# argmaxinc/WhisperKit

Measured on NVIDIA H100. Metric: RTFx (audio-sec/s) whisper-large-v3 greedy, higher is better.
Workload: dtype bf16

## Files before the change

### include/wkb200.h

```cpp
#ifndef WKB200_H
#define WKB200_H

#include <stdint.h>

#ifdef __cplusplus
extern "C" {
#endif

typedef int32_t wk_status;
enum {
    WK_OK = 0,
    WK_ERR_INVALID_ARGUMENT = -1,
    WK_ERR_MODELS_UNAVAILABLE = -2,
    WK_ERR_AUDIO_PROCESSING_FAILED = -3,
    WK_ERR_PREPARE_DECODER_INPUTS = -4,
    WK_ERR_DECODING_LOGITS_FAILED = -5,
    WK_ERR_DECODING_FAILED = -6,
    WK_ERR_TRANSCRIPTION_FAILED = -7,
    WK_ERR_CUDA = -8
};

typedef struct wk_model wk_model;
typedef struct wk_session wk_session;
typedef struct wk_tensor wk_tensor;
// ... 250 lines not shown
int32_t wk_write_srt(const float* starts, const float* ends, const char* const* texts, int32_t n, char* out, int32_t cap);
int32_t wk_write_vtt(const float* starts, const float* ends, const char* const* texts, int32_t n, char* out, int32_t cap);

int64_t wk_kernel_launch_count(int32_t reset);
wk_status wk_last_timings(wk_model* m, float* ms6);
void* wk_model_stream(wk_model* m);

wk_status wk_test_gemm(wk_model* m, const void* a, const void* w, const float* bias, void* out, int32_t M, int32_t N, int32_t K,
                       int32_t in_dtype, int32_t out_dtype, int32_t gelu);
wk_status wk_test_gemm_residual(wk_model* m, const void* a, const void* w, const float* bias, float* out, int32_t M, int32_t N, int32_t K, int32_t in_dtype);
wk_status wk_test_gemm_splitk(wk_model* m, const void* w, const void* x, float* out, int32_t N, int32_t rows_x, int32_t K, int32_t in_dtype, int32_t splits);
wk_status wk_test_attention(wk_model* m, const void* qkv, void* out, int32_t B, int32_t T, int32_t n_heads, int32_t dtype);
wk_status wk_test_cross_attention(wk_model* m, const float* q, const void* kcross, const void* vcross, void* out, int32_t B, int32_t H,
                                  int32_t T, int32_t dtype, const int32_t* done);
wk_status wk_test_cross_attention_shared(wk_model* m, const float* q, const void* kcross, const void* vcross, void* out, int32_t B, int32_t H,
                                         int32_t T, int32_t dtype, const int32_t* done, int32_t kv_div);
wk_status wk_test_cross_attention_fp8(wk_model* m, const float* q, const uint8_t* kcodes, const uint8_t* vcodes, const float* kscale,
                                      const float* vscale, void* out, int32_t B, int32_t H, int32_t T, int32_t dtype, const int32_t* done,
                                      int32_t kv_div, float* align_out);
wk_status wk_test_self_attention(wk_model* m, const float* qkv, void* kcache, void* vcache, const int32_t* pos, void* out, int32_t B,
                                 int32_t H, int32_t dtype, const int32_t* done);
wk_status wk_test_gemm_partial(wk_model* m, const void* w, const void* x, float* partial_out, int32_t N, int32_t rows_x, int32_t partial_cols,
                               int32_t K, int32_t dtype, int32_t splits);
wk_status wk_test_decoder_reduce(wk_model* m, int32_t kind, const float* partial, int32_t splits, int32_t Bp, const float* bias, const float* gamma,
                                 const float* beta, float* x, void* out16, int32_t B, int32_t n, int32_t dtype);
wk_status wk_test_self_attention_splitk(wk_model* m, const float* partial, int32_t splits, int32_t Bp, const float* bq, const float* bv, void* kcache,
                                        void* vcache, const int32_t* pos, const int32_t* done, const int32_t* anc, void* out, int32_t B, int32_t H,
                                        int32_t dtype);
wk_status wk_test_cross_attention_splitk(wk_model* m, const float* partial, int32_t splits, int32_t Bp, const float* bq, const void* kcross,
                                         const void* vcross, const float* kscale, const float* vscale, void* out, int32_t B, int32_t H, int32_t T,
                                         int32_t dtype, const int32_t* done, int32_t kv_div);

wk_status wk_bench_kernel(wk_model* m, wk_session* s, int32_t which, int32_t batch, int32_t iters, float* ms_out, double* work_out);

wk_status wk_debug_read(wk_model* m, wk_session* s, int32_t which, int64_t offset_elems, float* dst, int64_t n);

#ifdef __cplusplus
}
#endif
#endif
```

### whisperkit_b200/_lib.py

```python
from __future__ import annotations

import ctypes as C
import os

_PKG = os.path.dirname(os.path.abspath(__file__))
LIB_PATH = os.path.join(_PKG, "libwkb200.so")

WK_DTYPE_F32, WK_DTYPE_F16, WK_DTYPE_BF16, WK_DTYPE_I32 = 0, 1, 2, 3
WK_DTYPE_FP8_E4M3 = 4

STATUS_NAMES = {
    0: "ok", -1: "invalidArgument", -2: "modelsUnavailable", -3: "audioProcessingFailed",
    -4: "prepareDecoderInputsFailed", -5: "decodingLogitsFailed", -6: "decodingFailed",
    -7: "transcriptionFailed", -8: "cudaError",
}


class WhisperError(RuntimeError):

    def __init__(self, status: int, message: str):
        super().__init__(f"{STATUS_NAMES.get(status, status)}: {message}")
        self.status = status
        self.case = STATUS_NAMES.get(status, str(status))

# ... 172 lines not shown
    ("wk_tokenizer_vocab_size", I32, [P]),
    ("wk_tokenizer_token_to_id", I32, [P, C.c_char_p]),
    ("wk_tokenizer_decode", I32, [P, PI32, I32, I32, C.POINTER(C.c_char), I32]),
    ("wk_tokenizer_encode", I32, [P, C.c_char_p, PI32, I32]),
    ("wk_tokenizer_set_merges", I32, [P, C.POINTER(C.c_char_p), C.POINTER(C.c_char_p), I32]),
    ("wk_tokenizer_special_tokens", I32, [P, C.POINTER(wk_special_tokens)]),
    ("wk_tokenizer_split_to_word_tokens", I32, [P, PI32, I32, C.POINTER(C.c_char), I32, PI32, I32]),
    ("wk_tokenizer_hooks_init", I32, [P, C.POINTER(wk_tokenizer_hooks)]),
    ("wk_format_time", I32, [F32, I32, C.c_char_p, C.POINTER(C.c_char), I32]),
    ("wk_write_srt", I32, [PF32, PF32, C.POINTER(C.c_char_p), I32, C.POINTER(C.c_char), I32]),
    ("wk_write_vtt", I32, [PF32, PF32, C.POINTER(C.c_char_p), I32, C.POINTER(C.c_char), I32]),
    ("wk_kernel_launch_count", I64, [I32]),
    ("wk_last_timings", I32, [P, PF32]),
    ("wk_model_stream", P, [P]),
    ("wk_test_gemm", I32, [P, P, P, P, P, I32, I32, I32, I32, I32, I32]),
    ("wk_test_cross_attention", I32, [P, P, P, P, P, I32, I32, I32, I32, P]),
    ("wk_test_cross_attention_shared", I32, [P, P, P, P, P, I32, I32, I32, I32, P, I32]),
    ("wk_test_cross_attention_fp8", I32, [P, P, P, P, P, P, P, I32, I32, I32, I32, P, I32, P]),
    ("wk_test_self_attention", I32, [P, P, P, P, P, P, I32, I32, I32, P]),
    ("wk_test_gemm_residual", I32, [P, P, P, P, P, I32, I32, I32, I32]),
    ("wk_test_gemm_splitk", I32, [P, P, P, P, I32, I32, I32, I32, I32]),
    ("wk_test_attention", I32, [P, P, P, I32, I32, I32, I32]),
    ("wk_test_gemm_partial", I32, [P, P, P, P, I32, I32, I32, I32, I32, I32]),
    ("wk_test_decoder_reduce", I32, [P, I32, P, I32, I32, P, P, P, P, P, I32, I32, I32]),
    ("wk_test_self_attention_splitk", I32, [P, P, I32, I32, P, P, P, P, P, P, P, P, I32, I32, I32]),
    ("wk_test_cross_attention_splitk", I32, [P, P, I32, I32, P, P, P, P, P, P, I32, I32, I32, I32, P, I32]),
    ("wk_debug_read", I32, [P, P, I32, I64, P, I64]),
    ("wk_bench_kernel", I32, [P, P, I32, I32, I32, PF32, C.POINTER(C.c_double)]),
]

_lib = None


def load() -> C.CDLL:
    global _lib
    if _lib is not None:
        return _lib
    if not os.path.exists(LIB_PATH):
        raise ImportError(
            f"{LIB_PATH} not built: run `python -m whisperkit_b200.build` (needs nvcc). "
            "whisperkit_b200 has no CPU or PyTorch fallback.")
    lib = C.CDLL(LIB_PATH)
    for name, restype, argtypes in SYMBOLS:
        fn = getattr(lib, name)
        fn.restype = restype
        fn.argtypes = argtypes
# ... 8 lines not shown
```

### whisperkit_b200/csrc/decoder_ops.cu

```cuda
#include <curand_kernel.h>
#include <math.h>

#include <stdlib.h>

#include "common.cuh"
#include <algorithm>
#include "kernels.h"

namespace wk {

static constexpr int kMaxCtx = 224;

__device__ __forceinline__ float block_sum(float v, float* scratch) {
    v = warp_sum(v);
    const int warp = threadIdx.x >> 5, lane = threadIdx.x & 31, nw = (blockDim.x + 31) >> 5;
    __syncthreads();
    if (lane == 0) scratch[warp] = v;
    __syncthreads();
    float r = (lane < nw) ? scratch[lane] : 0.f;
    r = warp_sum(r);
    return r;
}
__device__ __forceinline__ float block_max(float v, float* scratch) {
    v = warp_max(v);
// ... 586 lines not shown
    launch_k(decoder_cross_attention_kernel<T, FP8>, dim3(B * H), dim3(kCrossThreads), cross_smem_bytes<FP8>(Tlen), stream, 4, partial, splits, Bp, bq,
             (const uint8_t*)kcross, (const uint8_t*)vcross, kscale, vscale, (T*)out, B, H, Tlen, done, align_scratch, align_mask, kv_div);
    return WK_OK;
}


__global__ void decoder_align_mean_kernel(const float* __restrict__ scratch, int n_slots, const int32_t* __restrict__ steps,
                                          const int32_t* __restrict__ done, const int32_t* __restrict__ lang_state, __half* __restrict__ out,
                                          int B, int Tlen, int max_rows) {
    const int b = blockIdx.y, t = blockIdx.x * blockDim.x + threadIdx.x;
    const int row = steps[b];
    if (t >= Tlen || row >= max_rows || done[b] || (lang_state != nullptr && lang_state[b] == kLangLeadRan)) return;
    float a = 0.f;
    for (int s = 0; s < n_slots; ++s) a += scratch[((long long)s * B + b) * Tlen + t];
    out[((long long)b * max_rows + row) * Tlen + t] = __float2half(a / (float)n_slots);
}

wk_status decoder_align_mean(const float* scratch, int n_slots, const int32_t* steps, const int32_t* done, const int32_t* lang_state,
                             void* out_f16, int B, int T, int max_rows, cudaStream_t stream) {
    launch_k(decoder_align_mean_kernel, dim3((T + 255) / 256, B), dim3(256), 0, stream, 0, scratch, n_slots, steps, done, lang_state, (__half*)out_f16, B, T, max_rows);
    count_launch();
    cudaError_t e = cudaGetLastError();
    if (e != cudaSuccess) { set_error("decoder_align_mean launch: %s", cudaGetErrorString(e)); return WK_ERR_CUDA; }
    return WK_OK;
}

wk_status decoder_cross_attention(const float* partial, int splits, int Bp, const float* bq, const void* kcross,
                                  const void* vcross, void* out, int B, int H, int T, int dtype, cudaStream_t stream,
                                  const int32_t* done, float* align_scratch, uint32_t align_mask, int kv_div, const float* kscale,
                                  const float* vscale) {
    const bool fp8 = kscale != nullptr;
    if (kv_div < 1 || B % kv_div != 0) { set_error("decoder_cross_attention: %d rows do not split into groups of %d", B, kv_div); return WK_ERR_INVALID_ARGUMENT; }
    if (!fp8 && T % kCrossRows != 0) { set_error("decoder_cross_attention: n_audio_ctx %d not a multiple of %d", T, kCrossRows); return WK_ERR_INVALID_ARGUMENT; }
    if (kv_div > 1 && kv_div <= 8 && align_scratch == nullptr)
        return decoder_cross_attention_mq(partial, splits, Bp, bq, kcross, vcross, out, B, H, T, dtype, stream, done, kv_div, kscale, vscale);
    if (fp8 && (T % CrossCfg<true>::kRows != 0 || T % 4 != 0)) { set_error("decoder_cross_attention (fp8): n_audio_ctx %d not a multiple of 500", T); return WK_ERR_INVALID_ARGUMENT; }
    const bool f16 = dtype == WK_DTYPE_F16;
    wk_status st = fp8 ? (f16 ? launch_cross<__half, true>(partial, splits, Bp, bq, kcross, vcross, kscale, vscale, out, B, H, T, stream, done, align_scratch, align_mask, kv_div)
                              : launch_cross<__nv_bfloat16, true>(partial, splits, Bp, bq, kcross, vcross, kscale, vscale, out, B, H, T, stream, done, align_scratch, align_mask, kv_div))
                       : (f16 ? launch_cross<__half, false>(partial, splits, Bp, bq, kcross, vcross, kscale, vscale, out, B, H, T, stream, done, align_scratch, align_mask, kv_div)
                              : launch_cross<__nv_bfloat16, false>(partial, splits, Bp, bq, kcross, vcross, kscale, vscale, out, B, H, T, stream, done, align_scratch, align_mask, kv_div));
    if (st != WK_OK) return st;
    count_launch();
    cudaError_t e = cudaGetLastError();
    if (e != cudaSuccess) { set_error("decoder_cross_attention launch: %s", cudaGetErrorString(e)); return WK_ERR_CUDA; }
    return WK_OK;
// ... 457 lines not shown
```

### whisperkit_b200/csrc/engine.cu

```cuda
#include <math.h>
#include <stdarg.h>
#include <stdio.h>
#include <stdlib.h>
#include <string.h>
#include <dirent.h>

#include <algorithm>
#include <atomic>
#include <map>
#include <string>
#include <vector>

#include "common.cuh"
#include "engine.h"

namespace wk {

static thread_local char g_err[1024] = "";
void set_error(const char* fmt, ...) {
    va_list ap;
    va_start(ap, fmt);
    vsnprintf(g_err, sizeof(g_err), fmt, ap);
    va_end(ap);
}
// ... 1022 lines not shown

wk_status wk_test_gemm_partial(wk_model* m, const void* w, const void* x, float* partial_out, int32_t N, int32_t rows_x, int32_t partial_cols,
                               int32_t K, int32_t dtype, int32_t splits) {
    if (!m || !w || !x || !partial_out || N < 1 || rows_x < 16 || rows_x > 256 || rows_x % 16 != 0 || partial_cols < 1 || partial_cols > rows_x ||
        splits < 1) {
        set_error("wk_test_gemm_partial: bad arguments");
        return WK_ERR_INVALID_ARGUMENT;
    }
    WK_CUDA_CHECK(cudaSetDevice(m->device));
    std::lock_guard<std::mutex> lock(m->api_mu);
    GemmDesc g;
    memset(&g, 0, sizeof(g));
    g.a = w; g.a_rows = N; g.a_cols = K; g.a_ld = K; g.a_batches = 1;
    g.b = x; g.b_rows = rows_x; g.b_ld = K; g.in_dtype = dtype;
    g.m_rows_per_batch = N; g.n = rows_x; g.k = K; g.taps = 1; g.bn = rows_x; g.splits = splits;
    g.mode = GEMM_OUT_PARTIAL_T; g.out = partial_out; g.ld_out = N; g.out_rows_per_batch = N; g.partial_cols = partial_cols;
    g.pdl = 1; g.a_static = 1;
    wk_status r = gemm_wgmma(g, m->num_sms, m->stream);
    cudaError_t e = cudaStreamSynchronize(m->stream);
    if (r == WK_OK && e != cudaSuccess) { set_error("wk_test_gemm_partial: %s", cudaGetErrorString(e)); r = WK_ERR_CUDA; }
    return r;
}

wk_status wk_test_decoder_reduce(wk_model* m, int32_t kind, const float* partial, int32_t splits, int32_t Bp, const float* bias, const float* gamma,
                                 const float* beta, float* x, void* out16, int32_t B, int32_t n, int32_t dtype) {
    if (!m || !partial || !out16 || B < 1 || Bp < B || splits < 1 || n < 4 || n % 4 != 0 || (kind == 0 && (!gamma || !beta || !x)) ||
        (kind == 1 && !bias) || kind < 0 || kind > 1) {
        set_error("wk_test_decoder_reduce: bad arguments");
        return WK_ERR_INVALID_ARGUMENT;
    }
    WK_CUDA_CHECK(cudaSetDevice(m->device));
    std::lock_guard<std::mutex> lock(m->api_mu);
    wk_status r = kind == 0 ? decoder_reduce_resid_ln(partial, splits, Bp, bias, gamma, beta, x, out16, B, n, dtype, m->stream)
                            : decoder_reduce_bias_gelu(partial, splits, Bp, bias, out16, B, n, dtype, m->stream);
    cudaError_t e = cudaStreamSynchronize(m->stream);
    if (r == WK_OK && e != cudaSuccess) { set_error("wk_test_decoder_reduce: %s", cudaGetErrorString(e)); r = WK_ERR_CUDA; }
    return r;
}

wk_status wk_test_self_attention_splitk(wk_model* m, const float* partial, int32_t splits, int32_t Bp, const float* bq, const float* bv, void* kcache,
                                        void* vcache, const int32_t* pos, const int32_t* done, const int32_t* anc, void* out, int32_t B, int32_t H,
                                        int32_t dtype) {
    if (!m || !partial || !bq || !bv || !kcache || !vcache || !pos || !out || B < 1 || Bp < B || splits < 1 || H < 1) {
        set_error("wk_test_self_attention_splitk: bad arguments");
        return WK_ERR_INVALID_ARGUMENT;
    }
// ... 27 lines not shown
```

### whisperkit_b200/csrc/gemm_wgmma.cu

```cuda
#include <stdarg.h>
#include <stdio.h>
#include <stdlib.h>

#include <algorithm>

#include "common.cuh"
#include "kernels.h"
#include "wgmma.cuh"

namespace wk {

static constexpr int kBlockM = 128;
static constexpr int kBlockK = 64;
static constexpr int kStageA = kBlockM * kBlockK * 2;
static constexpr int kGemmThreads = 384;
static constexpr int kMaxStages = 10;
static constexpr int kSmemMax = 227 * 1024;

struct GemmKParams {
    int tiles_per_batch, n_batches, tiles_n, splits, work;
    int kb_per_tap, kb_per_split, taps;
    int tap_row_shift[3];
    int tap_col_off[3];
    int a_is_3d;
// ... 339 lines not shown
        if constexpr (EPI == kEpiFp8Heads) {
            gemm_epilogue_fp8_heads<BN>(p, batch, tile_row0, r_lo, c_lo, col_base, acc);
        } else if constexpr (EPI == kEpiStore16) {
            if (wg_rows) gemm_epilogue_store16<T, BN>(p, &tmO, acc, my_stage, sbuf, wg_tid, cw, batch, wg_row0, col_base);
        } else if constexpr (EPI == kEpiStore32) {
            if (wg_rows) gemm_epilogue_store32<BN>(p, &tmO, acc, my_stage, my_res_bar, sbuf, rphase, wg_tid, cw, batch, wg_row0, col_base);
        } else {
            float* o = reinterpret_cast<float*>(p.out);
#pragma unroll
            for (int half = 0; half < 2; ++half) {
                const int row_in_batch = tile_row0 + r_lo + 8 * half;
                if (row_in_batch >= p.m_rows_per_batch) continue;
                const long long grow = (long long)batch * p.out_rows_per_batch + row_in_batch;
#pragma unroll
                for (int j = 0; j < BN / 8; ++j) {
                    const int col = col_base + 8 * j + c_lo;
                    if (col < p.partial_cols) o[((long long)split * p.partial_cols + col) * p.ld_out + grow] = acc[4 * j + 2 * half];
                    if (col + 1 < p.partial_cols) o[((long long)split * p.partial_cols + col + 1) * p.ld_out + grow] = acc[4 * j + 2 * half + 1];
                }
            }
        }
    }
    if (kStore && wg_tid == 0) bulk_wait_all();
}

typedef CUresult (*PFN_encodeTiled)(CUtensorMap*, CUtensorMapDataType, cuuint32_t, void*, const cuuint64_t*, const cuuint64_t*,
                                    const cuuint32_t*, const cuuint32_t*, CUtensorMapInterleave, CUtensorMapSwizzle,
                                    CUtensorMapL2promotion, CUtensorMapFloatOOBfill);

static PFN_encodeTiled get_encode_fn() {
    static PFN_encodeTiled fn = nullptr;
    if (!fn) {
        void* p = nullptr;
        cudaDriverEntryPointQueryResult q;
        if (cudaGetDriverEntryPoint("cuTensorMapEncodeTiled", &p, cudaEnableDefault, &q) == cudaSuccess &&
            q == cudaDriverEntryPointSuccess)
            fn = reinterpret_cast<PFN_encodeTiled>(p);
    }
    return fn;
}

static wk_status make_tmap(CUtensorMap* tm, const void* base, int dtype, int ndim, const uint64_t* dims,
                           const uint64_t* strides_bytes, const uint32_t* box) {
    PFN_encodeTiled enc = get_encode_fn();
    if (!enc) {
        set_error("cuTensorMapEncodeTiled entry point unavailable (no CUDA driver?)");
// ... 169 lines not shown
        const int out_dtype = epi == kEpiStore16 ? d.in_dtype : WK_DTYPE_F32;
        const uint64_t es = epi == kEpiStore16 ? 2 : 4;
        uint64_t dims[3] = {(uint64_t)d.n, (uint64_t)d.m_rows_per_batch, (uint64_t)p.n_batches};
        uint64_t str[2] = {(uint64_t)d.ld_out * es, (uint64_t)d.out_rows_per_batch * d.ld_out * es};
        uint32_t box[3] = {(uint32_t)(128 / es), 64, 1};
        st = make_tmap(&tmO, d.out, out_dtype, 3, dims, str, box);
    }
    if (st != WK_OK) return st;
    const size_t smem_bytes = (size_t)stages * stage_bytes + p.store_bytes + 1024 + 256;
    int grid = p.work < num_sms ? p.work : num_sms;
    if (grid < 1) return WK_OK;
    const int pdl = d.pdl != 0 ? 16 : 0;
    cudaError_t e = d.in_dtype == WK_DTYPE_F16 ? launch_gemm_n<__half>(tmA, tmB, tmO, p, grid, smem_bytes, pdl, stream)
                                               : launch_gemm_n<__nv_bfloat16>(tmA, tmB, tmO, p, grid, smem_bytes, pdl, stream);
    count_launch();
    if (e == cudaSuccess) e = cudaGetLastError();
    if (e != cudaSuccess) {
        set_error("gemm_wgmma launch: %s", cudaGetErrorString(e));
        return WK_ERR_CUDA;
    }
    return WK_OK;
}

}
```

### whisperkit_b200/csrc/kernels.h

```cpp
#pragma once
#include <cuda.h>
#include <cuda_runtime.h>
#include <stdint.h>

#include "../../include/wkb200.h"

namespace wk {

void set_error(const char* fmt, ...);
const char* last_error_cstr();
void count_launch(int n = 1);

enum GemmMode {
    GEMM_OUT_T16 = 0,
    GEMM_OUT_F32_ADD = 1,
    GEMM_OUT_F32_GELU_POS = 2,
    GEMM_OUT_PARTIAL_T = 3,
    GEMM_OUT_T16_HEADS = 4,
    GEMM_OUT_F32 = 5,
    GEMM_OUT_FP8_HEADS = 6,
};

struct GemmDesc {
    const void* a;
// ... 13 lines not shown
    int taps;
    int tap_row_shift[3];
    int tap_col_off[3];
    int bn;
    int splits;
    int mode;
    int gelu;
    void* out;
    int64_t ld_out;
    int64_t out_rows_per_batch;
    int64_t partial_cols;
    const float* bias;
    const float* pos;
    int64_t ld_pos;
    int heads_T, heads_B, heads_H, heads_dmodel;
    float* out_scale;
    int pdl;
    int max_stages;
    int a_static;
};

wk_status gemm_wgmma(const GemmDesc& d, int num_sms, cudaStream_t stream);
int wgmma_tile_n(int bn);

struct MelTables;
wk_status mel_tables_create(int n_mels, MelTables** out);
void mel_tables_free(MelTables* t);
wk_status mel_forward(const MelTables* t, const float* pcm, int64_t n_windows, int64_t stride, const int32_t* n_valid,
                      void* out_f16, int32_t* gmax_scratch, cudaStream_t stream);
constexpr int kMelRows = 3002;
constexpr int kMelCols = 128;

wk_status layernorm_f32_to_16(const float* x, const float* gamma, const float* beta, void* out, int64_t rows, int d, int dtype,
                              cudaStream_t stream);
wk_status layernorm_f32_to_f32(const float* x, const float* gamma, const float* beta, float* out, int64_t rows, int d,
                               cudaStream_t stream);
wk_status encoder_attention(const void* qkv, void* out, int B, int T, int n_heads, int dtype, cudaStream_t stream);
wk_status encoder_attention_wgmma(const void* qkv, void* out, int B, int T, int n_heads, int dtype, cudaStream_t stream);
wk_status transpose_to_host_layout(const void* src, float* dst, int64_t B, int64_t rows, int64_t cols, int64_t src_rows_alloc,
                                   int64_t src_row_off, int64_t src_ld, int dtype, cudaStream_t stream);
wk_status fill_random_16(void* dst, int64_t n, uint64_t seed, float std, float mean, int dtype, cudaStream_t stream);
wk_status fill_random_f32(float* dst, int64_t n, uint64_t seed, float std, float mean, cudaStream_t stream);
wk_status convert_to_16(const void* src, int src_dtype, void* dst, int dst_dtype, int64_t n, cudaStream_t stream);

struct RowParams {
    int32_t prompt_len;
// ... 54 lines not shown
    BeamState beam;
    int sample_begin_ts, sample_begin_blank, n_suppress;
    float temperature; int top_k; uint64_t seed;
};

wk_status decoder_embed_ln(const void* emb16, const float* pos, const float* gamma, const float* beta, DecodeState st, int vocab,
                           int ts_begin, float* x, void* xn, int B, int d, int dtype, const int32_t* explicit_pos, cudaStream_t stream);
wk_status decoder_reduce_resid_ln(const float* partial, int splits, int Bp, const float* bias, const float* gamma,
                                  const float* beta, float* x, void* xn, int B, int d, int dtype, cudaStream_t stream);
wk_status decoder_reduce_bias_gelu(const float* partial, int splits, int Bp, const float* bias, void* out, int B, int n,
                                   int dtype, cudaStream_t stream);
wk_status decoder_self_attention(const float* partial, int splits, int Bp, const float* bq, const float* bv, void* kcache,
                                 void* vcache, const int32_t* pos, const int32_t* done, void* out, int B, int H,
                                 int max_len, int dtype, cudaStream_t stream, const int32_t* anc = nullptr);
wk_status decoder_cross_attention(const float* partial, int splits, int Bp, const float* bq, const void* kcross,
                                  const void* vcross, void* out, int B, int H, int T, int dtype, cudaStream_t stream,
                                  const int32_t* done = nullptr, float* align_scratch = nullptr, uint32_t align_mask = 0, int kv_div = 1,
                                  const float* kscale = nullptr, const float* vscale = nullptr);
wk_status decoder_cross_attention_mq(const float* partial, int splits, int Bp, const float* bq, const void* kcross, const void* vcross, void* out, int B, int H,
                                     int Tlen, int dtype, cudaStream_t stream, const int32_t* done, int nq,
                                     const float* kscale = nullptr, const float* vscale = nullptr);
wk_status decoder_align_mean(const float* scratch, int n_slots, const int32_t* steps, const int32_t* done, const int32_t* lang_state,
                             void* out_f16, int B, int T, int max_rows, cudaStream_t stream);
wk_status sampler_filter_sample(const float* logits, int64_t ld_logits, SamplerParams p, DecodeState st, const int32_t* tokens,
                                int ld_tokens, const int32_t* n_tokens, int32_t* token_out, float* logprob_out,
                                float* filtered_out, int B, cudaStream_t stream);
wk_status decode_slots_init(DecodeState st, RowParams* rp_dev, const int32_t* slot_ids, const int32_t* prompts, const RowParams* rp_new,
                            int n, cudaStream_t stream, BeamState beam = BeamState());
wk_status beam_update(DecodeState st, BeamState beam, wk_special_tokens sp, int max_ctx, int groups, cudaStream_t stream);

wk_status align_embed(const void* emb, const float* pos_emb, const int32_t* row_tok, float* x, int64_t rows, int d, int dtype, cudaStream_t stream);
wk_status align_self_attention(const void* qkv, const int32_t* seq_len, void* out, int nw, int H, int dtype, cudaStream_t stream);
wk_status align_cross_attention(const void* q, const void* kc, const void* vc, const float* kscale, const float* vscale, const int32_t* seq_len,
                                int slot0, void* out, float* stats, int64_t stat_rows, int nw, int H, int Tlen, int dtype, cudaStream_t stream);
wk_status align_export(const void* q, const void* kc, const float* kscale, const float* stats, int64_t stat_rows, const int32_t* seq_len, int slot0,
                       uint32_t mask, int first, float* acc, int nw, int H, int Tlen, int dtype, cudaStream_t stream);
wk_status align_rows_f16(const float* acc, const int32_t* seq_len, int n_slots, void* out, int nw, int Tlen, int store_rows, cudaStream_t stream);
wk_status align_token_logprobs(const float* logits, int64_t ld, int64_t r0, int64_t rows, const int32_t* row_tok, const int32_t* seq_len, int eot,
                               float* out, cudaStream_t stream);

wk_status make_tmap_2d(void* tm, const void* base, int dtype, uint64_t cols, uint64_t rows, uint64_t ld_elems, uint32_t box_cols, uint32_t box_rows);
constexpr int kChainMaxPhases = 7;
constexpr int kChainMaxGemms = 4;
struct ChainPhaseDesc {
    int kind;
    const void* w; int n, k;
// ... 18 lines not shown
```

### whisperkit_b200/csrc/session.cu

```cuda
#include <math.h>
#include <stdio.h>
#include <stdlib.h>
#include <string.h>
#include <zlib.h>

#include <algorithm>
#include <string>
#include <vector>

#include "common.cuh"
#include "engine.h"

using namespace wk;

struct wk_session {
    wk_model* m = nullptr;
    int max_batch = 0;
    int batch = 0;
    int bound_windows = 0;
    int bp = 16;
    cudaStream_t stream = nullptr;
    cudaStream_t enc_stream = nullptr;
    EncWorkspace ws;
    void* cross_kv = nullptr;
// ... 6 lines not shown
    float* logits = nullptr;
    DecodeState st;
    RowParams* rp_dev = nullptr;
    int32_t* pos_dev = nullptr; int32_t* lang_dev = nullptr;
    int32_t* suppress_dev = nullptr; size_t suppress_cap = 0;
    int32_t *h_adm_slots = nullptr, *h_adm_prompts = nullptr; RowParams* h_adm_rp = nullptr;
    int32_t *d_adm_slots = nullptr, *d_adm_prompts = nullptr; RowParams* d_adm_rp = nullptr;
    int32_t *h_tokens = nullptr, *h_n_tokens = nullptr, *h_done = nullptr, *h_first_low = nullptr, *h_steps = nullptr, *h_error = nullptr;
    float* h_logprobs = nullptr;
    int32_t* h_lang_token = nullptr; float* h_lang_logprob = nullptr; float* h_no_speech = nullptr;
    std::vector<int32_t> win_lang; std::vector<float> win_lang_logprob;
    std::vector<float> win_no_speech;
    cudaGraphExec_t graph_exec = nullptr, graph_exec_live = nullptr;
    int graph_batch = 0; bool graph_align = false, graph_fused = false; wk_special_tokens graph_st; long long launches_per_step = 0;
    bool warmed = false;
    float* align_scratch = nullptr; void* align_w = nullptr; int align_slots = 0; bool align_on = false;
    void* align_store = nullptr; int64_t align_store_cap = 0, align_store_n = 0; int align_store_rows = kKvMaxLen;
    int al_cap = 0;
    float *al_acc = nullptr, *al_stats = nullptr, *al_lp = nullptr, *al_bqkv = nullptr;
    int32_t *al_tok = nullptr, *al_seq = nullptr;
    std::vector<float> win_align_lp;
    unsigned int* chain_counters = nullptr;
    cudaEvent_t ev_enc = nullptr, ev_adm = nullptr, ev_stage = nullptr, ev_t[10];
    bool knob_fused = false, knob_graph = true;
    BeamState bs = BeamState(); int bs_cap_rows = 0;
    int32_t *h_n_fin = nullptr, *h_fin_len = nullptr, *h_fin_tokens = nullptr; float *h_fin_score = nullptr, *h_fin_lps = nullptr, *h_sum_lp = nullptr;
    int graph_beam = 1;
    std::vector<int> slot_window, slot_try;
    int64_t stats[4] = {0, 0, 0, 0};
};

namespace wk {

static wk_status dec_gemm(wk_session* s, const void* w, int N, int K, const void* act, int* splits_out) {
    wk_model* m = s->m;
    GemmDesc g;
    memset(&g, 0, sizeof(g));
    g.a = w; g.a_rows = N; g.a_cols = K; g.a_ld = K; g.a_batches = 1;
    g.b = act; g.b_rows = s->bp; g.b_ld = K; g.in_dtype = m->cfg.dtype;
    g.m_rows_per_batch = N; g.n = s->bp; g.k = K; g.taps = 1; g.bn = s->bp;
    const int tiles = (N + 127) / 128;
    g.splits = choose_splits(tiles, K / 64, m->num_sms);
    g.mode = GEMM_OUT_PARTIAL_T; g.out = s->partial; g.ld_out = N; g.out_rows_per_batch = N; g.partial_cols = s->bp;
    g.pdl = 1; g.a_static = 1;
    if ((size_t)g.splits * s->bp * N > s->partial_elems) { set_error("partial workspace too small"); return WK_ERR_DECODING_FAILED; }
    *splits_out = g.splits;
    return gemm_wgmma(g, m->num_sms, s->stream);
}

static size_t ckv_esize(const wk_session* s) { return s->ckv_fp8 ? 1 : 2; }
static GemmDesc cross_kv_gemm(const wk_session* s, const void* src, int cnt, int q0) {
    const wk_model_config& c = s->m->cfg;
    const int T = c.n_audio_ctx, H = c.n_heads;
    GemmDesc g = plain_gemm(src, (int64_t)cnt * T, c.d_model, s->m->wckv, 2 * c.dec_layers * c.d_model, c.dtype,
                            s->ckv_fp8 ? GEMM_OUT_FP8_HEADS : GEMM_OUT_T16_HEADS, (char*)s->cross_kv + (size_t)q0 * H * T * 64 * ckv_esize(s), 0,
                            s->m->bckv, 0);
    g.heads_T = T; g.heads_B = s->max_batch; g.heads_H = H; g.heads_dmodel = c.d_model;
    if (s->ckv_fp8) g.out_scale = s->cross_scale + (size_t)q0 * H * T;
    return g;
}

static bool use_fused(const wk_session* s) { return s->knob_fused && s->m->live_sessions.load(std::memory_order_relaxed) == 1; }

static wk_status decoder_forward(wk_session* s, int ts_begin, const int32_t* explicit_pos, bool fused, bool check_done = true) {
    wk_model* m = s->m;
    const wk_model_config& c = m->cfg;
    const int d = c.d_model, H = c.n_heads, dt = c.dtype, B = s->batch, Bp = s->bp, T = c.n_audio_ctx;
    cudaStream_t st = s->stream;
    const size_t self_layer = (size_t)s->max_batch * H * kKvMaxLen * 64 * 2;
    const size_t cross_rows = (size_t)s->max_batch * H * T;
// ... 65 lines not shown
            WK_CHECK(dec_gemm(s, l.wqkv, 3 * d, d, s->xn, &sp));
            WK_CHECK(self_attn(li, l));
            WK_CHECK(dec_gemm(s, l.wo, d, d, s->attn, &sp));
            WK_CHECK(decoder_reduce_resid_ln(s->partial, sp, Bp, l.bo, l.lnx.g, l.lnx.b, s->x, s->xn, B, d, dt, st));
            WK_CHECK(dec_gemm(s, l.wcq, d, d, s->xn, &sp));
            WK_CHECK(cross_attn(li, l));
            WK_CHECK(dec_gemm(s, l.wco, d, d, s->attn, &sp));
            WK_CHECK(decoder_reduce_resid_ln(s->partial, sp, Bp, l.bco, l.ln3.g, l.ln3.b, s->x, s->xn, B, d, dt, st));
            WK_CHECK(dec_gemm(s, l.w1, 4 * d, d, s->xn, &sp));
            WK_CHECK(decoder_reduce_bias_gelu(s->partial, sp, Bp, l.b1, s->ffn, B, 4 * d, dt, st));
            WK_CHECK(dec_gemm(s, l.w2, d, 4 * d, s->ffn, &sp));
            const LayerNormW& nxt = (li + 1 < n_layers) ? m->dec[li + 1].ln1 : m->dec_ln;
            WK_CHECK(decoder_reduce_resid_ln(s->partial, sp, Bp, l.b2, nxt.g, nxt.b, s->x, s->xn, B, d, dt, st));
        }
    }
    {
        GemmDesc g;
        memset(&g, 0, sizeof(g));
        g.a = m->emb; g.a_rows = c.vocab; g.a_cols = d; g.a_ld = d; g.a_batches = 1;
        g.b = s->xn; g.b_rows = Bp; g.b_ld = d; g.in_dtype = dt;
        g.m_rows_per_batch = c.vocab; g.n = Bp; g.k = d; g.taps = 1; g.bn = Bp; g.splits = 1;
        g.mode = GEMM_OUT_PARTIAL_T; g.out = s->logits; g.ld_out = c.vocab; g.out_rows_per_batch = c.vocab; g.partial_cols = B;
        g.pdl = 1; g.a_static = 1;
        WK_CHECK(gemm_wgmma(g, m->num_sms, st));
    }
    return WK_OK;
}

static SamplerParams loop_sampler_params(wk_session* s, const wk_special_tokens* st) {
    SamplerParams p;
    memset(&p, 0, sizeof(p));
    p.st = *st;
    p.vocab = s->m->cfg.vocab;
    p.is_multilingual = s->m->cfg.vocab != 51864;
    p.loop_mode = 1;
    p.suppress = s->suppress_dev;
    p.max_ctx = kKvMaxLen;
    p.detect_tokens = s->lang_dev;
    p.beam = s->bs;
    return p;
}

static float compression_ratio(const std::vector<int32_t>& toks) {
    if (toks.empty()) return INFINITY;
    const uLong n = (uLong)toks.size() * 4;
    z_stream zs;
    memset(&zs, 0, sizeof(zs));
// ... 785 lines not shown
            slot0 = 0;
        }
        for (int i = 0; i < cnt; ++i) seq[i] = tokens + (len[w0 + i] > 0 ? offsets[w0 + i] : 0);
        WK_CHECK(align_chunk(s, st, slot0, cnt, w0, seq.data(), len.data() + w0));
    }
    s->align_on = true;
    if (!first_err.empty()) set_error("%s", first_err.c_str());
    return WK_OK;
}

}

extern "C" {

wk_status wk_session_create(wk_model* m, int32_t max_batch, wk_session** out) {
    if (!m || !out || max_batch < 1 || max_batch > 256) { set_error("wk_session_create: bad arguments (max_batch %d, limit 256)", max_batch); return WK_ERR_INVALID_ARGUMENT; }
    WK_CUDA_CHECK(cudaSetDevice(m->device));
    const wk_model_config& c = m->cfg;
    const int d = c.d_model, H = c.n_heads, L = c.dec_layers, T = c.n_audio_ctx, S = max_batch;
    wk_session* s = new wk_session();
    s->m = m;
    s->max_batch = S;
    if (const char* e = getenv("WKB200_FUSED")) s->knob_fused = atoi(e) != 0;
    s->knob_graph = getenv("WKB200_NO_GRAPH") == nullptr;
    WK_CUDA_CHECK(cudaStreamCreateWithFlags(&s->stream, cudaStreamNonBlocking));
    WK_CUDA_CHECK(cudaStreamCreateWithFlags(&s->enc_stream, cudaStreamNonBlocking));
    const int bpm = round_up(S, 16);
    {
        std::lock_guard<std::mutex> lock(m->api_mu);
        m->session_created = true;
        s->ckv_fp8 = m->cross_kv_fp8;
    }
    if (s->ckv_fp8) {
        uint8_t* codes = nullptr;
        WK_CHECK(dmalloc(&codes, (size_t)2 * L * S * H * T * 64));
        s->cross_kv = codes;
        WK_CHECK(dmalloc(&s->cross_scale, (size_t)2 * L * S * H * T));
    } else {
        WK_CHECK(alloc16(&s->cross_kv, (size_t)2 * L * S * H * T * 64));
    }
    WK_CHECK(alloc16(&s->self_k, (size_t)L * S * H * kKvMaxLen * 64));
    WK_CHECK(alloc16(&s->self_v, (size_t)L * S * H * kKvMaxLen * 64));
    size_t pe = 0;
    const int shapes[4][2] = {{3 * d, d}, {d, d}, {4 * d, d}, {d, 4 * d}};
    for (auto& sh : shapes) {
        const int sp = choose_splits((sh[0] + 127) / 128, sh[1] / 64, m->num_sms);
// ... 482 lines not shown
```

Before: 923.3.

## Add a specialized small-batch warp-specialized WGMMA GEMM for decoder split-K projections

Adds a dedicated decoder GEMM kernel (288 threads, one TMA producer warp, two consumer warpgroups, up to three blocks per SM) for the transposed-partial output mode with small batch widths up to 64. It is enabled by default through a session knob and replaces the generic wgmma GEMM for the decoder linear layers and the logits projection. The producer prefetches weight tiles before the PDL wait so the weight stream overlaps the previous kernel's tail. Test and footprint-query entry points are also added. The kernel does not use the wrapper's `s` stream for the logits GEMM (it uses s->stream instead of st), which could differ if st is another stream.

```diff
diff --git a/include/wkb200.h b/include/wkb200.h
--- a/include/wkb200.h
+++ b/include/wkb200.h
@@ -296,6 +296,9 @@
                                  int32_t H, int32_t dtype, const int32_t* done);
 wk_status wk_test_gemm_partial(wk_model* m, const void* w, const void* x, float* partial_out, int32_t N, int32_t rows_x, int32_t partial_cols,
                                int32_t K, int32_t dtype, int32_t splits);
+wk_status wk_test_dec_gemm_partial(wk_model* m, const void* w, const void* x, float* partial_out, int32_t N, int32_t rows_x, int32_t partial_cols,
+                                   int32_t K, int32_t dtype, int32_t splits, int32_t kernel);
+wk_status wk_test_dec_gemm_footprint(wk_model* m, int64_t* out);
 wk_status wk_test_decoder_reduce(wk_model* m, int32_t kind, const float* partial, int32_t splits, int32_t Bp, const float* bias, const float* gamma,
                                  const float* beta, float* x, void* out16, int32_t B, int32_t n, int32_t dtype);
 wk_status wk_test_self_attention_splitk(wk_model* m, const float* partial, int32_t splits, int32_t Bp, const float* bq, const float* bv, void* kcache,
diff --git a/whisperkit_b200/_lib.py b/whisperkit_b200/_lib.py
--- a/whisperkit_b200/_lib.py
+++ b/whisperkit_b200/_lib.py
@@ -218,6 +218,8 @@
     ("wk_test_gemm_splitk", I32, [P, P, P, P, I32, I32, I32, I32, I32]),
     ("wk_test_attention", I32, [P, P, P, I32, I32, I32, I32]),
     ("wk_test_gemm_partial", I32, [P, P, P, P, I32, I32, I32, I32, I32, I32]),
+    ("wk_test_dec_gemm_partial", I32, [P, P, P, P, I32, I32, I32, I32, I32, I32, I32]),
+    ("wk_test_dec_gemm_footprint", I32, [P, P]),
     ("wk_test_decoder_reduce", I32, [P, I32, P, I32, I32, P, P, P, P, P, I32, I32, I32]),
     ("wk_test_self_attention_splitk", I32, [P, P, I32, I32, P, P, P, P, P, P, P, P, I32, I32, I32]),
     ("wk_test_cross_attention_splitk", I32, [P, P, I32, I32, P, P, P, P, P, P, I32, I32, I32, I32, P, I32]),
diff --git a/whisperkit_b200/csrc/decoder_ops.cu b/whisperkit_b200/csrc/decoder_ops.cu
--- a/whisperkit_b200/csrc/decoder_ops.cu
+++ b/whisperkit_b200/csrc/decoder_ops.cu
@@ -632,6 +632,22 @@
     count_launch();
     cudaError_t e = cudaGetLastError();
     if (e != cudaSuccess) { set_error("decoder_align_mean launch: %s", cudaGetErrorString(e)); return WK_ERR_CUDA; }
+    return WK_OK;
+}
+
+wk_status decoder_kernel_footprints(int Tlen, int64_t* out) {
+    struct K { const void* f; int threads; size_t dyn; };
+    const K ks[4] = {{(const void*)decoder_cross_attention_kernel<__nv_bfloat16, false>, kCrossThreads, cross_smem_bytes<false>(Tlen)},
+                     {(const void*)decoder_self_attention_kernel<__nv_bfloat16, false>, 128, 0},
+                     {(const void*)decoder_reduce_resid_ln_kernel<__nv_bfloat16>, kReduceThreads, 0},
+                     {(const void*)decoder_reduce_bias_gelu_kernel<__nv_bfloat16>, 256, 0}};
+    for (int i = 0; i < 4; ++i) {
+        cudaFuncAttributes a;
+        WK_CUDA_CHECK(cudaFuncGetAttributes(&a, ks[i].f));
+        out[3 * i] = a.numRegs;
+        out[3 * i + 1] = ks[i].threads;
+        out[3 * i + 2] = (int64_t)a.sharedSizeBytes + (int64_t)ks[i].dyn;
+    }
     return WK_OK;
 }
 
diff --git a/whisperkit_b200/csrc/engine.cu b/whisperkit_b200/csrc/engine.cu
--- a/whisperkit_b200/csrc/engine.cu
+++ b/whisperkit_b200/csrc/engine.cu
@@ -1068,6 +1068,46 @@
     return r;
 }
 
+wk_status wk_test_dec_gemm_partial(wk_model* m, const void* w, const void* x, float* partial_out, int32_t N, int32_t rows_x, int32_t partial_cols,
+                                   int32_t K, int32_t dtype, int32_t splits, int32_t kernel) {
+    if (!m || !w || !x || !partial_out || N < 1 || rows_x < 16 || rows_x > 256 || rows_x % 16 != 0 || partial_cols < 1 || partial_cols > rows_x ||
+        splits < 1 || kernel < 0 || kernel > 1 || (kernel == 1 && !dec_gemm_supported(rows_x))) {
+        set_error("wk_test_dec_gemm_partial: bad arguments");
+        return WK_ERR_INVALID_ARGUMENT;
+    }
+    WK_CUDA_CHECK(cudaSetDevice(m->device));
+    std::lock_guard<std::mutex> lock(m->api_mu);
+    GemmDesc g;
+    memset(&g, 0, sizeof(g));
+    g.a = w; g.a_rows = N; g.a_cols = K; g.a_ld = K; g.a_batches = 1;
+    g.b = x; g.b_rows = rows_x; g.b_ld = K; g.in_dtype = dtype;
+    g.m_rows_per_batch = N; g.n = rows_x; g.k = K; g.taps = 1; g.bn = rows_x; g.splits = splits;
+    g.mode = GEMM_OUT_PARTIAL_T; g.out = partial_out; g.ld_out = N; g.out_rows_per_batch = N; g.partial_cols = partial_cols;
+    g.pdl = 1; g.a_static = 1;
+    wk_status r = kernel == 1 ? dec_gemm_wgmma(g, m->num_sms, m->stream) : gemm_wgmma(g, m->num_sms, m->stream);
+    cudaError_t e = cudaStreamSynchronize(m->stream);
+    if (r == WK_OK && e != cudaSuccess) { set_error("wk_test_dec_gemm_partial: %s", cudaGetErrorString(e)); r = WK_ERR_CUDA; }
+    return r;
+}
+
+wk_status wk_test_dec_gemm_footprint(wk_model* m, int64_t* out) {
+    if (!m || !out) { set_error("wk_test_dec_gemm_footprint: bad arguments"); return WK_ERR_INVALID_ARGUMENT; }
+    WK_CUDA_CHECK(cudaSetDevice(m->device));
+    memset(out, 0, 24 * sizeof(int64_t));
+    int regs = 0, local = 0, ssmem = 0, maxt = 0;
+    WK_CHECK(dec_gemm_attributes(&regs, &local, &ssmem, &maxt));
+    out[0] = regs; out[1] = dec_gemm_threads(); out[2] = ssmem + (int64_t)dec_gemm_smem_bytes(64, 2); out[3] = local;
+    int64_t f[12];
+    WK_CHECK(decoder_kernel_footprints(1500, f));
+    for (int i = 0; i < 4; ++i) { out[4 * (i + 1)] = f[3 * i]; out[4 * (i + 1) + 1] = f[3 * i + 1]; out[4 * (i + 1) + 2] = f[3 * i + 2]; }
+    int v = 0;
+    WK_CUDA_CHECK(cudaDeviceGetAttribute(&v, cudaDevAttrMaxSharedMemoryPerMultiprocessor, m->device)); out[20] = v;
+    WK_CUDA_CHECK(cudaDeviceGetAttribute(&v, cudaDevAttrMaxRegistersPerMultiprocessor, m->device)); out[21] = v;
+    WK_CUDA_CHECK(cudaDeviceGetAttribute(&v, cudaDevAttrReservedSharedMemoryPerBlock, m->device)); out[22] = v;
+    WK_CUDA_CHECK(cudaDeviceGetAttribute(&v, cudaDevAttrMaxThreadsPerMultiProcessor, m->device)); out[23] = v;
+    return WK_OK;
+}
+
 wk_status wk_test_decoder_reduce(wk_model* m, int32_t kind, const float* partial, int32_t splits, int32_t Bp, const float* bias, const float* gamma,
                                  const float* beta, float* x, void* out16, int32_t B, int32_t n, int32_t dtype) {
     if (!m || !partial || !out16 || B < 1 || Bp < B || splits < 1 || n < 4 || n % 4 != 0 || (kind == 0 && (!gamma || !beta || !x)) ||
diff --git a/whisperkit_b200/csrc/gemm_wgmma.cu b/whisperkit_b200/csrc/gemm_wgmma.cu
--- a/whisperkit_b200/csrc/gemm_wgmma.cu
+++ b/whisperkit_b200/csrc/gemm_wgmma.cu
@@ -385,6 +385,124 @@
         }
     }
     if (kStore && wg_tid == 0) bulk_wait_all();
+}
+
+static constexpr int kDecThreads = 288;
+static constexpr int kDecMaxBN = 64;
+
+template <typename T, int BN>
+__global__ void __launch_bounds__(kDecThreads, 3)
+dec_gemm_kernel(const __grid_constant__ CUtensorMap tmA, const __grid_constant__ CUtensorMap tmB, const GemmKParams p) {
+    extern __shared__ __align__(1024) uint8_t smem_raw[];
+    uint8_t* smem = reinterpret_cast<uint8_t*>((reinterpret_cast<uintptr_t>(smem_raw) + 1023) & ~uintptr_t(1023));
+    const int stage_bytes = kStageA + p.stage_b_bytes;
+    uint64_t* full_bar = reinterpret_cast<uint64_t*>(smem + (size_t)p.stages * stage_bytes);
+    uint64_t* empty_bar = full_bar + kMaxStages;
+
+    const int warp = threadIdx.x >> 5;
+    const int lane = threadIdx.x & 31;
+    pdl_launch_dependents();
+
+    if (warp == 8 && lane == 0) {
+        tma_prefetch_desc(&tmA);
+        tma_prefetch_desc(&tmB);
+        for (int i = 0; i < p.stages; ++i) {
+            mbar_init(&full_bar[i], 1);
+            mbar_init(&empty_bar[i], 8);
+        }
+        fence_barrier_init();
+    }
+    __syncthreads();
+
+    if (warp == 8) {
+        int stage = 0;
+        uint32_t phase = 0;
+        bool need_wait = true;
+        auto issue = [&](int kb, int st, int row0, int n_tile, bool do_a, bool do_b) {
+            uint8_t* sa = smem + (size_t)st * stage_bytes;
+            if (do_a) {
+                mbar_expect_tx_elect(&full_bar[st], (uint32_t)stage_bytes);
+                tma_load_2d_elect(sa, &tmA, &full_bar[st], kb * kBlockK, row0);
+            }
+            if (do_b) tma_load_2d_elect(sa + kStageA, &tmB, &full_bar[st], kb * kBlockK, n_tile * BN);
+        };
+        for (int w = blockIdx.x; w < p.work; w += gridDim.x) {
+            const int split = w % p.splits;
+            const int t = w / p.splits;
+            const int n_tile = t % p.tiles_n;
+            const int row0 = (t / p.tiles_n) * kBlockM;
+            const int kb0 = split * p.kb_per_split;
+            int kb = kb0;
+            if (need_wait) {
+                const int n_pre = p.kb_per_split < p.stages ? p.kb_per_split : p.stages;
+                for (int i = 0; i < n_pre; ++i) issue(kb0 + i, i, row0, n_tile, true, false);
+                pdl_wait();
+                for (int i = 0; i < n_pre; ++i) issue(kb0 + i, i, row0, n_tile, false, true);
+                kb = kb0 + n_pre;
+                if (n_pre == p.stages) { stage = 0; phase ^= 1; } else stage = n_pre;
+                need_wait = false;
+            }
+            for (; kb < kb0 + p.kb_per_split; ++kb) {
+                mbar_wait(&empty_bar[stage], phase ^ 1);
+                __syncwarp();
+                issue(kb, stage, row0, n_tile, true, true);
+                if (++stage == p.stages) { stage = 0; phase ^= 1; }
+            }
+        }
+        if (need_wait) pdl_wait();
+        return;
+    }
+
+    pdl_wait();
+    const int cw = warp >> 2;
+    const int r_lo = cw * 64 + (warp & 3) * 16 + (lane >> 2);
+    const int c_lo = 2 * (lane & 3);
+    int stage = 0;
+    uint32_t phase = 0;
+    float acc[BN / 2];
+    for (int w = blockIdx.x; w < p.work; w += gridDim.x) {
+        const int split = w % p.splits;
+        const int t = w / p.splits;
+        const int n_tile = t % p.tiles_n;
+        const int tile_row0 = (t / p.tiles_n) * kBlockM;
+        const int col_base = n_tile * BN;
+
+        int prev = -1;
+        for (int kb = 0; kb < p.kb_per_split; ++kb) {
+            mbar_wait(&full_bar[stage], phase);
+            const uint32_t sa = smem_u32(smem + (size_t)stage * stage_bytes);
+            const uint64_t adesc = wgmma_desc_sw128(sa + cw * 64 * 128);
+            const uint64_t bdesc = wgmma_desc_sw128(sa + kStageA);
+            wgmma_fence();
+#pragma unroll
+            for (int k = 0; k < kBlockK / 16; ++k)
+                Wgmma<T, BN>::ss(acc, adesc + (uint64_t)(2 * k), bdesc + (uint64_t)(2 * k), (kb > 0 || k > 0) ? 1u : 0u);
+            wgmma_commit();
+            wgmma_wait<1>();
+            if (prev >= 0) {
+                __syncwarp();
+                if (lane == 0) mbar_arrive(&empty_bar[prev]);
+            }
+            prev = stage;
+            if (++stage == p.stages) { stage = 0; phase ^= 1; }
+        }
+        wgmma_wait<0>();
+        __syncwarp();
+        if (lane == 0) mbar_arrive(&empty_bar[prev]);
+
+        float* o = reinterpret_cast<float*>(p.out);
+#pragma unroll
+        for (int half = 0; half < 2; ++half) {
+            const int row = tile_row0 + r_lo + 8 * half;
+            if (row >= p.m_rows_per_batch) continue;
+#pragma unroll
+            for (int j = 0; j < BN / 8; ++j) {
+                const int col = col_base + 8 * j + c_lo;
+                if (col < p.partial_cols) o[((long long)split * p.partial_cols + col) * p.ld_out + row] = acc[4 * j + 2 * half];
+                if (col + 1 < p.partial_cols) o[((long long)split * p.partial_cols + col + 1) * p.ld_out + row] = acc[4 * j + 2 * half + 1];
+            }
+        }
+    }
 }
 
 typedef CUresult (*PFN_encodeTiled)(CUtensorMap*, CUtensorMapDataType, cuuint32_t, void*, const cuuint64_t*, const cuuint64_t*,
@@ -600,4 +718,118 @@
     return WK_OK;
 }
 
-}
+static int dec_gemm_stage_bytes(int bn) { return kStageA + (bn * kBlockK * 2 + 1023) / 1024 * 1024; }
+static int dec_gemm_stages(int bn, int kb_per_split) {
+    int stages = (kSmemMax - 1024 - 256) / dec_gemm_stage_bytes(bn);
+    if (stages > kMaxStages) stages = kMaxStages;
+    if (stages > kb_per_split + 2) stages = kb_per_split + 2;
+    return stages < 2 ? 2 : stages;
+}
+size_t dec_gemm_smem_bytes(int bn, int kb_per_split) {
+    const int tn = wgmma_tile_n(bn);
+    return (size_t)dec_gemm_stages(tn, kb_per_split) * dec_gemm_stage_bytes(tn) + 1024  + 256 ;
+}
+bool dec_gemm_supported(int bn) { return bn >= 1 && bn <= kDecMaxBN; }
+
+template <typename T, int BN>
+static cudaError_t launch_dec_gemm(const CUtensorMap& tmA, const CUtensorMap& tmB, const GemmKParams& p, int grid, size_t smem, int pdl,
+                                   cudaStream_t stream) {
+    static bool attr_set = false;
+    if (!attr_set) {
+        const cudaError_t e = cudaFuncSetAttribute(dec_gemm_kernel<T, BN>, cudaFuncAttributeMaxDynamicSharedMemorySize, kSmemMax);
+        if (e != cudaSuccess) return e;
+        attr_set = true;
+    }
+    return launch_k(dec_gemm_kernel<T, BN>, dim3(grid), dim3(kDecThreads), smem, stream, pdl, tmA, tmB, p);
+}
+
+template <typename T>
+static cudaError_t launch_dec_gemm_n(const CUtensorMap& tmA, const CUtensorMap& tmB, const GemmKParams& p, int grid, size_t smem, int pdl,
+                                     cudaStream_t stream) {
+    switch (p.bn) {
+        case 16: return launch_dec_gemm<T, 16>(tmA, tmB, p, grid, smem, pdl, stream);
+        case 32: return launch_dec_gemm<T, 32>(tmA, tmB, p, grid, smem, pdl, stream);
+        default: return launch_dec_gemm<T, 64>(tmA, tmB, p, grid, smem, pdl, stream);
+    }
+}
+
+wk_status dec_gemm_wgmma(const GemmDesc& d, int num_sms, cudaStream_t stream) {
+    if (d.mode != GEMM_OUT_PARTIAL_T || d.taps != 1 || d.a_3d || d.k % kBlockK != 0 || d.bn % 16 != 0 || !dec_gemm_supported(d.bn)) {
+        set_error("dec_gemm_wgmma: unsupported GEMM (mode %d taps %d k %d bn %d)", d.mode, d.taps, d.k, d.bn);
+        return WK_ERR_INVALID_ARGUMENT;
+    }
+    GemmKParams p;
+    memset(&p, 0, sizeof(p));
+    const int total_kb = d.k / kBlockK;
+    p.splits = d.splits < 1 ? 1 : d.splits;
+    if (total_kb % p.splits != 0) {
+        set_error("dec_gemm_wgmma: splits %d does not divide %d k-blocks", p.splits, total_kb);
+        return WK_ERR_INVALID_ARGUMENT;
+    }
+    p.kb_per_split = total_kb / p.splits;
+    p.kb_per_tap = total_kb;
+    p.taps = 1;
+    p.n_batches = 1;
+    p.m_rows_per_batch = d.m_rows_per_batch;
+    p.tiles_per_batch = (d.m_rows_per_batch + kBlockM - 1) / kBlockM;
+    p.n = d.n;
+    p.bn = wgmma_tile_n(d.bn);
+    p.tiles_n = (d.n + p.bn - 1) / p.bn;
+    p.work = p.tiles_per_batch * p.tiles_n * p.splits;
+    p.stage_b_bytes = dec_gemm_stage_bytes(p.bn) - kStageA;
+    p.stages = dec_gemm_stages(p.bn, p.kb_per_split);
+    p.a_static = 1;
+    p.mode = d.mode;
+    p.out = d.out;
+    p.ld_out = d.ld_out;
+    p.out_rows_per_batch = d.out_rows_per_batch;
+    p.partial_cols = d.partial_cols;
+
+    CUtensorMap tmA, tmB;
+    {
+        uint64_t dims[2] = {(uint64_t)d.a_cols, (uint64_t)d.a_rows};
+        uint64_t str[1] = {(uint64_t)d.a_ld * 2};
+        uint32_t box[2] = {kBlockK, kBlockM};
+        const wk_status st = make_tmap(&tmA, d.a, d.in_dtype, 2, dims, str, box);
+        if (st != WK_OK) return st;
+    }
+    {
+        uint64_t dims[2] = {(uint64_t)d.k, (uint64_t)d.b_rows};
+        uint64_t str[1] = {(uint64_t)d.b_ld * 2};
+        uint32_t box[2] = {kBlockK, (uint32_t)p.bn};
+        const wk_status st = make_tmap(&tmB, d.b, d.in_dtype, 2, dims, str, box);
+        if (st != WK_OK) return st;
+    }
+    const size_t smem_bytes = dec_gemm_smem_bytes(p.bn, p.kb_per_split);
+    const int grid = std::min(p.work, num_sms);
+    if (grid < 1) return WK_OK;
+    const int pdl = d.pdl != 0 ? 16 : 0;
+    cudaError_t e = d.in_dtype == WK_DTYPE_F16 ? launch_dec_gemm_n<__half>(tmA, tmB, p, grid, smem_bytes, pdl, stream)
+                                               : launch_dec_gemm_n<__nv_bfloat16>(tmA, tmB, p, grid, smem_bytes, pdl, stream);
+    count_launch();
+    if (e == cudaSuccess) e = cudaGetLastError();
+    if (e != cudaSuccess) {
+        set_error("dec_gemm_wgmma launch: %s", cudaGetErrorString(e));
+        return WK_ERR_CUDA;
+    }
+    return WK_OK;
+}
+
+wk_status dec_gemm_attributes(int* regs, int* local_bytes, int* static_smem, int* max_threads) {
+    const void* fns[6] = {(const void*)dec_gemm_kernel<__nv_bfloat16, 16>, (const void*)dec_gemm_kernel<__nv_bfloat16, 32>,
+                          (const void*)dec_gemm_kernel<__nv_bfloat16, 64>, (const void*)dec_gemm_kernel<__half, 16>,
+                          (const void*)dec_gemm_kernel<__half, 32>, (const void*)dec_gemm_kernel<__half, 64>};
+    *regs = 0; *local_bytes = 0; *static_smem = 0; *max_threads = 1 << 30;
+    for (const void* f : fns) {
+        cudaFuncAttributes a;
+        WK_CUDA_CHECK(cudaFuncGetAttributes(&a, f));
+        *regs = std::max(*regs, a.numRegs);
+        *local_bytes = std::max(*local_bytes, (int)a.localSizeBytes);
+        *static_smem = std::max(*static_smem, (int)a.sharedSizeBytes);
+        *max_threads = std::min(*max_threads, a.maxThreadsPerBlock);
+    }
+    return WK_OK;
+}
+int dec_gemm_threads() { return kDecThreads; }
+
+}
diff --git a/whisperkit_b200/csrc/kernels.h b/whisperkit_b200/csrc/kernels.h
--- a/whisperkit_b200/csrc/kernels.h
+++ b/whisperkit_b200/csrc/kernels.h
@@ -59,6 +59,11 @@
 
 wk_status gemm_wgmma(const GemmDesc& d, int num_sms, cudaStream_t stream);
 int wgmma_tile_n(int bn);
+wk_status dec_gemm_wgmma(const GemmDesc& d, int num_sms, cudaStream_t stream);
+bool dec_gemm_supported(int bn);
+size_t dec_gemm_smem_bytes(int bn, int kb_per_split);
+int dec_gemm_threads();
+wk_status dec_gemm_attributes(int* regs, int* local_bytes, int* static_smem, int* max_threads);
 
 struct MelTables;
 wk_status mel_tables_create(int n_mels, MelTables** out);
@@ -159,6 +164,7 @@
                                      const float* kscale = nullptr, const float* vscale = nullptr);
 wk_status decoder_align_mean(const float* scratch, int n_slots, const int32_t* steps, const int32_t* done, const int32_t* lang_state,
                              void* out_f16, int B, int T, int max_rows, cudaStream_t stream);
+wk_status decoder_kernel_footprints(int Tlen, int64_t* out);
 wk_status sampler_filter_sample(const float* logits, int64_t ld_logits, SamplerParams p, DecodeState st, const int32_t* tokens,
                                 int ld_tokens, const int32_t* n_tokens, int32_t* token_out, float* logprob_out,
                                 float* filtered_out, int B, cudaStream_t stream);
diff --git a/whisperkit_b200/csrc/session.cu b/whisperkit_b200/csrc/session.cu
--- a/whisperkit_b200/csrc/session.cu
+++ b/whisperkit_b200/csrc/session.cu
@@ -52,7 +52,7 @@
     std::vector<float> win_align_lp;
     unsigned int* chain_counters = nullptr;
     cudaEvent_t ev_enc = nullptr, ev_adm = nullptr, ev_stage = nullptr, ev_t[10];
-    bool knob_fused = false, knob_graph = true;
+    bool knob_fused = false, knob_graph = true, knob_dec_gemm = true;
     BeamState bs = BeamState(); int bs_cap_rows = 0;
     int32_t *h_n_fin = nullptr, *h_fin_len = nullptr, *h_fin_tokens = nullptr; float *h_fin_score = nullptr, *h_fin_lps = nullptr, *h_sum_lp = nullptr;
     int graph_beam = 1;
@@ -61,6 +61,11 @@
 };
 
 namespace wk {
+
+static wk_status launch_dec_gemm(const wk_session* s, const GemmDesc& g) {
+    if (s->knob_dec_gemm && dec_gemm_supported(g.bn)) return dec_gemm_wgmma(g, s->m->num_sms, s->stream);
+    return gemm_wgmma(g, s->m->num_sms, s->stream);
+}
 
 static wk_status dec_gemm(wk_session* s, const void* w, int N, int K, const void* act, int* splits_out) {
     wk_model* m = s->m;
@@ -75,7 +80,7 @@
     g.pdl = 1; g.a_static = 1;
     if ((size_t)g.splits * s->bp * N > s->partial_elems) { set_error("partial workspace too small"); return WK_ERR_DECODING_FAILED; }
     *splits_out = g.splits;
-    return gemm_wgmma(g, m->num_sms, s->stream);
+    return launch_dec_gemm(s, g);
 }
 
 static size_t ckv_esize(const wk_session* s) { return s->ckv_fp8 ? 1 : 2; }
@@ -187,7 +192,7 @@
         g.m_rows_per_batch = c.vocab; g.n = Bp; g.k = d; g.taps = 1; g.bn = Bp; g.splits = 1;
         g.mode = GEMM_OUT_PARTIAL_T; g.out = s->logits; g.ld_out = c.vocab; g.out_rows_per_batch = c.vocab; g.partial_cols = B;
         g.pdl = 1; g.a_static = 1;
-        WK_CHECK(gemm_wgmma(g, m->num_sms, st));
+        WK_CHECK(launch_dec_gemm(s, g));
     }
     return WK_OK;
 }
@@ -1019,6 +1024,7 @@
     s->m = m;
     s->max_batch = S;
     if (const char* e = getenv("WKB200_FUSED")) s->knob_fused = atoi(e) != 0;
+    if (const char* e = getenv("WKB200_DEC_GEMM")) s->knob_dec_gemm = atoi(e) != 0;
     s->knob_graph = getenv("WKB200_NO_GRAPH") == nullptr;
     WK_CUDA_CHECK(cudaStreamCreateWithFlags(&s->stream, cudaStreamNonBlocking));
     WK_CUDA_CHECK(cudaStreamCreateWithFlags(&s->enc_stream, cudaStreamNonBlocking));
```

New measurement: 924.7, median of 6. No clear change (+0.2%).
